# GuanxingLu/ManiGaussian

Measured on AMD Instinct MI355X. Metric: Gaussians rasterized/sec (fwd+bwd), 128x128, 32 feat-ch; HBM GB/s vs peak, higher is better.
Workload: dtype f32

## Files before the change

manigaussian_amd/csrc/mgs_render_dense.hip:

```cpp
#include "mgs_render_common.h"

namespace mgs {

constexpr int TRACE_EVENTS = 24;
__device__ unsigned long long g_trace[512 * 16 * TRACE_EVENTS];
#define MGS_TRACE(ev)                                                                                      \
  do {                                                                                                     \
    if ((r.dbg & 256) && lane == 0 && blockIdx.x < 512 && (ev) < TRACE_EVENTS)                              \
      g_trace[((size_t)blockIdx.x * 16 + w) * TRACE_EVENTS + (ev)] = __builtin_amdgcn_s_memtime();         \
  } while (0)

template <int F, bool FAST, bool EXACT, int NW, int CHS, bool TWO>
__global__ void __launch_bounds__(NW * 64, TWO ? 4 : 1)
coop_fwd_pairs_kernel(RenderArgs r, const uint2* __restrict__ ranges, const uint32_t* __restrict__ point_list,
                      float* __restrict__ T_end, float* __restrict__ T_mid,
                      uint32_t* __restrict__ last_pos, float* __restrict__ partial, uint32_t* __restrict__ surv,
                      size_t surv_stride, uint2* __restrict__ nsurv, float* __restrict__ final_T,
                      uint32_t* __restrict__ last_chunk, float* __restrict__ out_color, float* __restrict__ out_feat,
                      uint32_t* __restrict__ round_base, uint32_t pool, uint32_t* __restrict__ flags, int nblocks,
                      uint64_t* host_status, uint32_t status_tag, unsigned long long* hs_fail_mark) {
  static_assert(CHS == 64, "a chunk is two 32-lane groups of the Gaussian-major backward");
  using f32x16 = __attribute__((ext_vector_type(16))) float;
  constexpr int NCH = F + 3;
  constexpr bool MF = F >= 16;
  constexpr int NT = MF ? (F + 31) / 32 : 0;
  constexpr int NVF = MF ? 0 : F;
  constexpr int NP = NW / 2;
  constexpr int NS = 2;
  constexpr int NSTEP = CHS / 2;
  constexpr int TRS = 33;
  constexpr int NOWN = (NCH + NW - 1) / NW;
  constexpr uint32_t ROUND = NW * CHS;
  constexpr uint32_t FSTEP = NW * 64;
  constexpr int FILLK = 3;
  constexpr int TRR = NT * 32 + 3;
  __shared__ float trs[MF ? NW * TRR * TRS : 1];
  __shared__ uint32_t lastcc[NW];
  __shared__ float4 recP[NW][CHS / 4 * 2 * 3];
  __shared__ uint32_t sid[NW * CHS];
  __shared__ float4 rowq[NW][NS][CHS];
  __shared__ float rowf[NVF > 0 ? NW * NS * CHS * NVF : 1];
  __shared__ float Tp[2][NW][64];
  __shared__ unsigned long long red_last[64];
  __shared__ uint32_t cnt[2][FILLK * NW];
  __shared__ uint32_t rbase[2];
  constexpr uint32_t RBH = 16;
  __shared__ uint32_t rb_hist[RBH];
  const int tid = threadIdx.x, lane = tid & 63;
  const int w = __builtin_amdgcn_readfirstlane(tid >> 6);
  if (blockIdx.x == 0 && tid == 0 && hs_fail_mark) *hs_fail_mark = 0ull;
  const int pr = w >> 1, hh = w & 1;
  const int k_ = lane >> 5, pl_ = lane & 31;
  int tile, sub;
  map_block(blockIdx.x, tile, sub);
  if (tile >= r.tiles_x * r.tiles_y) return;
  const PixBlk p = pix_blk(r, tile, sub, lane);
  const int pixq_ = 32 * hh + pl_;
  const int pixq = pixq_, k = k_, pl = pl_;
  const PixBlk pq = pix_blk(r, tile, sub, pixq);
  const int pixx_ = 32 * (hh ^ k) + pl;
  const int pixx = pixx_;
  const bool insidex = pix_blk(r, tile, sub, pixx).inside;
  const uint2 rng = ranges[tile];
  const bool use_feat = (F > 0) && r.include_feature;
  const bool eager = (r.dbg & (1 << 17)) != 0;
  const auto feat_rsrc = __builtin_amdgcn_make_buffer_rsrc(const_cast<float*>(r.feats), 0, 0xffffffffu, 0x00020000);
  uint32_t* __restrict__ my_rounds = round_base + round_entry(rng.x, tile, sub, 0);
  bool overflow = false;
  uint32_t* my_surv = surv + (size_t)sub * surv_stride + rng.x;

  float Tround = 1.0f;
  uint32_t my_vis = 0;
  float my_Tf = 1.0f;
  if (w == 0) red_last[lane] = (unsigned long long)__float_as_uint(1.0f);
  uint32_t my_lastcc = 0xffffffffu;
  MGS_TRACE(0);

  uint32_t next = rng.x;
  uint32_t qhead = 0;
  uint32_t qtail = 0;
  uint32_t cbase = 0;
  uint32_t fill = 0;
  uint32_t round = 0;

  const bool allocator = tid == (NW - 1) * 64;
  const bool static0 = (uint32_t)nblocks <= 1024u && (uint32_t)nblocks * (uint32_t)NW <= pool;
  const uint32_t dyn_base = static0 ? (uint32_t)nblocks * (uint32_t)NW : 0u;
  for (;; round++) {
    int k = k_, pl = pl_, pixq = pixq_, pixx = pixx_;
    asm volatile("" : "+v"(k), "+v"(pl), "+v"(pixq), "+v"(pixx));
    uint32_t b0 = 0;
    const bool more = next < rng.y || qtail > qhead;
    if (allocator && more) {
      if (static0 && round == 0) b0 = ((uint32_t)tile * 4u + (uint32_t)sub) * (uint32_t)NW;
      else b0 = dyn_base + atomicAdd(&flags[FLAG_CHUNKS_USED], (uint32_t)NW);
    }
    while (qtail - qhead < ROUND && next < rng.y) {
      uint32_t idd[FILLK], rk[FILLK];
      float4 a0[FILLK], a1[FILLK];
      {
#pragma unroll
        for (int kf = 0; kf < FILLK; kf++) {
          const uint32_t e = next + (uint32_t)kf * FSTEP + (uint32_t)tid;
          idd[kf] = e < rng.y ? point_list[e] : 0xffffffffu;
        }
#pragma unroll
        for (int kf = 0; kf < FILLK; kf++) {
          a0[kf] = make_float4(0, 0, 0, 0); a1[kf] = make_float4(0, 0, -1.f, -1.f);
          if (idd[kf] != 0xffffffffu) { a0[kf] = r.rec[2 * (size_t)idd[kf]]; a1[kf] = r.rec[2 * (size_t)idd[kf] + 1]; }
        }
#pragma unroll
        for (int kf = 0; kf < FILLK; kf++) {
          const bool sk = idd[kf] != 0xffffffffu && cull_ok<EXACT>(a0[kf], a1[kf], p);
          const unsigned long long sm = ballot(sk);
          rk[kf] = sk ? (uint32_t)__builtin_popcountll(sm & ((1ull << lane) - 1ull)) : 0xffffffffu;
          if (lane == 0) cnt[fill & 1][kf * NW + w] = (uint32_t)__builtin_popcountll(sm);
        }
      }
      __syncthreads();
      const uint32_t v = lane < FILLK * NW ? cnt[fill & 1][lane] : 0u;
      const uint32_t incl = wave_incl_scan_add_u32(v);
      const uint32_t total = bcast_lane_u32(incl, 63);
#pragma unroll
      for (int kf = 0; kf < FILLK; kf++) {
        const uint32_t base = bcast_lane_u32(incl - v, kf * NW + w);
        if (rk[kf] != 0xffffffffu) {
          const uint32_t n = qtail + base + rk[kf];
          my_surv[n] = idd[kf];
          if (round == 0 && n < ROUND) {
            const uint32_t e = n & (CHS - 1);
            float* rp = reinterpret_cast<float*>(&recP[n / CHS][0]) + (((e >> 2) * 2 + (e & 1)) * 12 + ((e >> 1) & 1));
            rp[0] = a0[kf].x; rp[2] = a0[kf].y; rp[4] = a0[kf].z; rp[6] = a0[kf].w; rp[8] = a1[kf].x; rp[10] = a1[kf].y;
            sid[n] = idd[kf];
          }
        }
      }
      qtail += total;
      next += FILLK * FSTEP;
      fill++;
    }
    if (allocator && more) {
      rbase[round & 1] = b0;
      if (round < RBH) rb_hist[round] = b0;
      my_rounds[4 * (size_t)round] = b0;
    }
    MGS_TRACE(1 + 8 * round);
    __syncthreads();
    MGS_TRACE(2 + 8 * round);
    const uint32_t avail = qtail - qhead;
    const bool exhausted = !(next < rng.y);
    uint32_t nchunk = exhausted ? (avail + CHS - 1) / CHS : avail / CHS;
    nchunk = min(nchunk, (uint32_t)NW);
    if (nchunk == 0) break;

    struct Rec3 { float4 XY, CC, ZO; };
    auto rec3_of = [&](uint32_t buf, int j) -> Rec3 {
      return Rec3{recP[buf][(2 * j + k) * 3], recP[buf][(2 * j + k) * 3 + 1], recP[buf][(2 * j + k) * 3 + 2]};
    };
    auto alpha2_rec = [&](const Rec3& R) -> f32x2 {
      const float4 XY = R.XY, CC = R.CC, ZO = R.ZO;
      const f32x2 dx = f32x2{XY.x, XY.y} - pq.pxf, dy = f32x2{XY.z, XY.w} - pq.pyf;
      const f32x2 power = gauss_power2v(f32x2{CC.x, CC.y}, f32x2{CC.z, CC.w}, f32x2{ZO.x, ZO.y}, dx, dy);
      const f32x2 G = exp2_<FAST>(power);
      const f32x2 oG = f32x2{ZO.z, ZO.w} * G;
      const float a0 = fminf(0.99f, oG.x), a1 = fminf(0.99f, oG.y);
      return f32x2{((power.x > 0.0f) || (a0 < 1.0f / 255.0f)) ? 0.f : a0, ((power.y > 0.0f) || (a1 < 1.0f / 255.0f)) ? 0.f : a1};
    };
    float al[NSTEP];
    uint32_t nmy[NS];
#pragma unroll
    for (int q = 0; q < NS; q++) {
      const uint32_t ci = (uint32_t)pr + (uint32_t)q * NP;
      nmy[q] = ci < nchunk ? min((uint32_t)CHS, avail - ci * CHS) : 0u;
    }
    auto phase_a = [&](const int q, const bool publish) __attribute__((always_inline)) {
      const uint32_t ci = (uint32_t)pr + (uint32_t)q * NP;
      const bool hasq = ci < nchunk;
      float tp = 1.0f;
      if (hasq) {
        float4 rq = make_float4(0, 0, 0, __uint_as_float(0u));
        float fv[NVF > 0 ? NVF : 1];
#pragma unroll
        for (int i = 0; i < (NVF > 0 ? NVF : 1); i++) fv[i] = 0.f;
        const bool valid = (uint32_t)lane < (q ? nmy[1] : nmy[0]);
        float* rp = reinterpret_cast<float*>(&recP[ci][0]) + (((lane >> 2) * 2 + (lane & 1)) * 12 + ((lane >> 1) & 1));
        int tile_ = tile;
        asm volatile("" : "+s"(tile_));
        const uint32_t gbase = gauss_base(r, tile_);
        auto colour_row = [&](uint32_t id) {
          const uint32_t gid = gauss_of(gbase, id);
          const uint32_t cid = r.colors_per_view ? id : gid;
          rq = make_float4(r.colors[(size_t)cid * 3], r.colors[(size_t)cid * 3 + 1], r.colors[(size_t)cid * 3 + 2],
                           __uint_as_float(gid));
          if constexpr (NVF > 0) {
            if (use_feat) {
#pragma unroll
              for (int i = 0; i < NVF; i++) fv[i] = r.feats[(size_t)gid * F + i];
            }
          }
        };
        if (round == 0) {
          if (valid) {
            colour_row(sid[ci * CHS + (uint32_t)lane]);
          } else {
            rp[0] = 0.f; rp[2] = 0.f; rp[4] = 0.f; rp[6] = 0.f; rp[8] = 0.f; rp[10] = 0.f;
            rq.w = __uint_as_float(gauss_of(gbase, sid[ci * CHS]));
          }
        } else {
          float4 g0 = make_float4(0, 0, 0, 0), g1 = make_float4(0, 0, -1.f, -1.f);
          if (valid) {
            const uint32_t id = my_surv[qhead + ci * CHS + (uint32_t)lane];
            g0 = r.rec[2 * (size_t)id]; g1 = r.rec[2 * (size_t)id + 1];
            colour_row(id);
          } else {
            rq.w = __uint_as_float(gauss_of(gbase, my_surv[qhead + ci * CHS]));
          }
          rp[0] = g0.x; rp[2] = g0.y; rp[4] = g0.z; rp[6] = g0.w; rp[8] = g1.x;
          rp[10] = valid ? g1.y : 0.f;
        }
        wave_lds_sync();
        if (q == 0) MGS_TRACE(3 + 8 * round);
        f32x2 tp2 = {1.0f, 1.0f};
        Rec3 Rn = rec3_of(ci, 0);
#pragma unroll
        for (int j = 0; j < NSTEP / 2; j++) {
          const Rec3 Rc = Rn;
          if (j + 1 < NSTEP / 2) Rn = rec3_of(ci, j + 1);
          const f32x2 a2 = alpha2_rec(Rc);
          al[2 * j] = a2.x; al[2 * j + 1] = a2.y;
          tp2 = tp2 * (1.0f - a2);
        }
        tp = tp2.x * tp2.y;
        rowq[w][q][lane] = rq;
        if constexpr (NVF > 0) {
#pragma unroll
          for (int i = 0; i < NVF; i++) rowf[(((size_t)w * NS + q) * CHS + lane) * NVF + i] = fv[i];
        }
        float t0 = tp, t1 = tp;
        swap32(t0, t1);
        tp = t0 * t1;
      }
      if (publish && k == 0) Tp[round & 1][ci][pixq] = tp;
    };
    uint32_t rb = 0;
    auto phase_b = [&](const int q, const float Tin_q) __attribute__((always_inline)) {
      const uint32_t ci = (uint32_t)pr + (uint32_t)q * NP;
      const bool hasq = ci < nchunk;
      const float Tpart = __uint_as_float(lane_xor<32>(__float_as_uint(Tin_q), lane));
      float T = k ? Tpart : Tin_q;
      const bool live = hasq && pq.inside && !(T < 0.0001f);
      if (ballot(live) != 0) {
        const uint32_t n_my = q ? nmy[1] : nmy[0];
        float Cc[3] = {0.f, 0.f, 0.f};
        float Cv[NVF > 0 ? NVF : 1];
#pragma unroll
        for (int i = 0; i < (NVF > 0 ? NVF : 1); i++) Cv[i] = 0.f;
        f32x16 acc[NT > 0 ? NT : 1];
#pragma unroll
        for (int t = 0; t < (NT > 0 ? NT : 1); t++)
#pragma unroll
          for (int i = 0; i < 16; i++) acc[t][i] = 0.f;
        constexpr int BD = 4;
        float Bq[NT > 0 ? NT : 1][BD];
        uint32_t gnext = __float_as_uint(rowq[w][q][k].w);
        auto load_B = [&](int s) {
          const uint32_t gide = gnext;
          if (s + 1 < NSTEP) gnext = __float_as_uint(rowq[w][q][2 * (s + 1) + k].w);
#pragma unroll
          for (int t = 0; t < (NT > 0 ? NT : 1); t++) {
            const int ch = 32 * t + pl;
            if constexpr (MF)
              Bq[t][s % BD] = __uint_as_float(__builtin_amdgcn_raw_buffer_load_b32(
                  feat_rsrc, gide * (uint32_t)(F * 4) + (uint32_t)((ch < F ? ch : 0) * 4), 0, 0));
          }
        };
        if constexpr (MF) {
#pragma unroll
          for (int s = 0; s < BD; s++) load_B(s);
        }
        float Tc = live ? T : 0.f;
        uint32_t last = 0;
        float Tm = T;
        bool stop = false;
        constexpr int GS = 4;
#pragma unroll
        for (int g = 0; g < NSTEP / GS; g++) {
          if (g * GS == NSTEP / 2) Tm = T;
          stop = stop || (uint32_t)(2 * g * GS) >= n_my || ballot(Tc != 0.f) == 0;
          __builtin_amdgcn_sched_barrier(0);
          if (!stop) {
#pragma unroll
            for (int u4 = 0; u4 < GS; u4++) {
              const int s = g * GS + u4;
              float a0 = al[s], a1 = a0;
              swap32(a0, a1);
              float wq[2];
              const float aa[2] = {a0, a1};
#pragma unroll
              for (int u = 0; u < 2; u++) {
                const float test_T = Tc * (1.0f - aa[u]);
                const bool term = test_T < 0.0001f;
                wq[u] = (term ? 0.f : aa[u]) * Tc;
                Tc = term ? 0.f : test_T;
                T = term ? T : test_T;
                last = wq[u] > 0.f ? (uint32_t)(2 * s + u) + 1u : last;
              }
              const float wk = k ? wq[1] : wq[0];
              const float4 rq = rowq[w][q][2 * s + k];
              Cc[0] += rq.x * wk; Cc[1] += rq.y * wk; Cc[2] += rq.z * wk;
              if constexpr (NVF > 0) {
#pragma unroll
                for (int i = 0; i < NVF; i++) Cv[i] += rowf[(((size_t)w * NS + q) * CHS + 2 * s + k) * NVF + i] * wk;
              }
              if constexpr (MF) {
#pragma unroll
                for (int t = 0; t < NT; t++) {
                  float bv = Bq[t][s % BD];
                  if constexpr (F % 32 != 0) bv = (32 * t + pl) < F ? bv : 0.f;
                  acc[t] = __builtin_amdgcn_mfma_f32_32x32x2f32(wk, bv, acc[t], 0, 0, 0);
                }
                if (s + BD < NSTEP) load_B(s + BD);
              }
            }
          }
        }
        if constexpr (MF) {
#pragma unroll
          for (int t = 0; t < NT; t++)
#pragma unroll
            for (int i = 0; i < BD; i++) asm volatile("" ::"v"(Bq[t][i]));
        }
        if (last <= 32u) Tm = T;
#pragma unroll
        for (int i = 0; i < 3; i++) Cc[i] += __uint_as_float(lane_xor<32>(__float_as_uint(Cc[i]), lane));
#pragma unroll
        for (int i = 0; i < NVF; i++) Cv[i] += __uint_as_float(lane_xor<32>(__float_as_uint(Cv[i]), lane));
        MGS_TRACE(6 + 8 * round);
        const size_t slot = (size_t)rb + (size_t)ci;
        float* pp = partial + slot * NCH * 64 + pixq;
        if (k == 0) {
          T_end[slot * 64 + pixq] = T;
          T_mid[slot * 64 + pixq] = Tm;
          last_pos[slot * 64 + pixq] = last;
#pragma unroll
          for (int i = 0; i < 3; i++) pp[i * 64] = Cc[i];
#pragma unroll
          for (int i = 0; i < NVF; i++) pp[(3 + i) * 64] = Cv[i];
        }
        if constexpr (MF) {
          float* tb = trs + (size_t)w * TRR * TRS;
#pragma unroll
          for (int t = 0; t < NT; t++)
#pragma unroll
            for (int i = 0; i < 16; i++)
              tb[(32 * t + pl) * TRS + (i & 3) + 8 * (i >> 2) + 4 * k] = acc[t][i];
          if (k == 0) {
#pragma unroll
            for (int i = 0; i < 3; i++) tb[(NT * 32 + i) * TRS + pl] = Cc[i];
          }
          wave_lds_sync();
#pragma unroll
          for (int c = 0; c < F / 2; c++) {
            const int ch = k * (F / 2) + c;
            pp[(3 + ch) * 64] = tb[ch * TRS + pl];
          }
          wave_lds_sync();
          my_lastcc = cbase + ci;
        }
        if (live) { my_vis = cbase + ci + 1; my_Tf = T; }
      }
    };
    constexpr int GA = 2;
    static_assert(GA < NP, "slot 1 goes in two groups of pairs");
    float Tnext = Tround;
    int p0 = 0, p1 = NP;
#pragma clang loop unroll(disable)
    for (int st = eager ? -1 : 0;; st++) {
      asm volatile("" : "+v"(k), "+v"(pl), "+v"(pixq), "+v"(pixx));
      const int q = st == 0 ? 0 : 1;
      const bool act = pr >= p0 && pr < p1;
#pragma unroll
      for (int s = 0; s < NSTEP; s++) al[s] = 0.f;
      if (act) {
        phase_a(q, st <= 0 || !eager);
        if (st > 0) MGS_TRACE(8 + 8 * round);
      }
      if (st < 0) continue;
      if (st == 0) MGS_TRACE(4 + 8 * round);
      if (st == 0 || !eager) __syncthreads();
      if (st == 0) {
        __builtin_amdgcn_s_waitcnt(0x0F70);
        MGS_TRACE(5 + 8 * round);
        rb = rbase[round & 1];
        if (rb + (uint32_t)NW > pool) { overflow = true; break; }
      }
      float Tin = Tnext;
#pragma unroll
      for (int c2 = 0; c2 < NP; c2++) {
        const float t2 = (c2 >= p0 && c2 < p1) ? Tp[round & 1][q * NP + c2][pixx] : 1.0f;
        Tin = (c2 < pr) ? Tin * t2 : Tin;
        Tnext *= t2;
      }
      if (act) phase_b(q, Tin);
      if (st == 2) break;
      p0 = st == 0 ? 0 : GA;
      p1 = st == 0 ? GA : NP;
      if (!((uint32_t)(NP + p0) < nchunk) || ballot(insidex && !(Tnext < 0.0001f)) == 0) break;
    }
    if (overflow) break;
    MGS_TRACE(7 + 8 * round);
    Tround = Tnext;
    qhead += min(avail, nchunk * CHS);
    cbase += nchunk;
    if (ballot(insidex && !(Tround < 0.0001f)) == 0) break;
  }

  MGS_TRACE(TRACE_EVENTS - 3);
  if (my_vis > 0 && k == 0)
    atomicMax(&red_last[pixq], ((unsigned long long)my_vis << 32) | (unsigned long long)__float_as_uint(my_Tf));
  if constexpr (MF) { if (lane == 0) lastcc[w] = my_lastcc; }
  __syncthreads();
  const unsigned long long rl = red_last[lane];
  const uint32_t vis = (uint32_t)(rl >> 32);
  const float Tf = __uint_as_float((uint32_t)rl);
  float img[NOWN];
#pragma unroll
  for (int kk = 0; kk < NOWN; kk++) img[kk] = 0.f;
  const uint32_t vmax = wave_umax(vis);
  constexpr int NFLY = 8;
  static_assert(NW % NFLY == 0, "a batch of the final sum lies inside one round");
  for (uint32_t c0 = 0; c0 < vmax; c0 += NFLY) {
    float v[NFLY][NOWN];
    const uint32_t rr = c0 / NW;
    uint32_t rb0 = rb_hist[rr < RBH ? rr : 0u];
    if (__builtin_expect(rr >= RBH, 0))
      rb0 = __hip_atomic_load(&my_rounds[4 * (size_t)rr], __ATOMIC_RELAXED, __HIP_MEMORY_SCOPE_WORKGROUP);
    rb0 = (uint32_t)__builtin_amdgcn_readfirstlane((int)rb0);
    bool inl[NFLY];
    unsigned long long needg = 0ull;
#pragma unroll
    for (int u = 0; u < NFLY; u++) {
      const uint32_t cc = c0 + u;
      inl[u] = false;
      if constexpr (MF) {
        const uint32_t ws = 2u * ((cc % NW) % NP) + (uint32_t)(lane >> 5);
        inl[u] = lastcc[ws] == cc;
      }
      needg |= ballot(cc < vis && !inl[u]);
#pragma unroll
      for (int kk = 0; kk < NOWN; kk++) v[u][kk] = 0.f;
    }
    if (needg != 0ull) {
#pragma unroll
      for (int u = 0; u < NFLY; u++) {
        const uint32_t cc = c0 + u;
        const bool gl = cc < vis && !inl[u];
        const size_t slot = gl ? (size_t)rb0 + (cc % NW) : 0;
        const float* pp = partial + slot * NCH * 64 + lane;
#pragma unroll
        for (int kk = 0; kk < NOWN; kk++) {
          const int ch = w + kk * NW;
          if (gl && ch < NCH && (ch < 3 || use_feat)) v[u][kk] = pp[ch * 64];
        }
      }
#pragma unroll
      for (int u = 0; u < NFLY; u++)
#pragma unroll
        for (int kk = 0; kk < NOWN; kk++) asm volatile("" : "+v"(v[u][kk]));
    }
    if constexpr (MF) {
#pragma unroll
      for (int u = 0; u < NFLY; u++) {
        const uint32_t cc = c0 + u;
        const uint32_t ws = 2u * ((cc % NW) % NP) + (uint32_t)(lane >> 5);
        const float* tb = trs + (size_t)ws * TRR * TRS + (lane & 31);
#pragma unroll
        for (int kk = 0; kk < NOWN; kk++) {
          const int ch = w + kk * NW;
          const int row = ch < 3 ? NT * 32 + ch : ch - 3;
          if (cc < vis && inl[u] && ch < NCH && (ch < 3 || use_feat)) v[u][kk] = tb[row * TRS];
        }
      }
    }
#pragma unroll
    for (int u = 0; u < NFLY; u++)
#pragma unroll
      for (int kk = 0; kk < NOWN; kk++) img[kk] += v[u][kk];
  }
  MGS_TRACE(TRACE_EVENTS - 2);
  uint32_t ticket = 0;
  if (tid == 0) {
    const uint32_t dep = overflow ? (atomicOr(&flags[FLAG_PREFILTERED], 0x100u) & 0u) : 0u;
    ticket = atomicAdd(&flags[FLAG_BLOCKS_DONE], 1u + dep) + 1u;
  }
  const size_t HW = (size_t)r.Hv * r.W;
  int lane_o = lane;
  asm volatile("" : "+v"(lane_o));
  const PixBlk po = pix_blk(r, tile, sub, lane_o);
  if (po.inside) {
#pragma unroll
    for (int kk = 0; kk < NOWN; kk++) {
      const int ch = w + kk * NW;
      if (ch < 3) out_color[((size_t)po.v * 3 + ch) * HW + po.pixl] = img[kk] + Tf * r.bg[ch];
      else if (ch < NCH && use_feat) out_feat[((size_t)po.v * F + (ch - 3)) * HW + po.pixl] = img[kk];
    }
  }
  if (w == 0) {
    last_chunk[((size_t)tile * 4 + sub) * 64 + lane] = vis;
    if (po.inside) final_T[po.pixa] = Tf;
    if (lane == 0) {
      nsurv[(size_t)tile * 4 + sub] = make_uint2(qtail, round > 0 || vis > 0 ? rb_hist[0] : 0u);
      if (ticket == (uint32_t)nblocks && host_status) {
        const uint32_t used = dyn_base + __hip_atomic_load(&flags[FLAG_CHUNKS_USED], __ATOMIC_RELAXED, __HIP_MEMORY_SCOPE_AGENT);
        const uint32_t ovf = (__hip_atomic_load(&flags[FLAG_PREFILTERED], __ATOMIC_RELAXED, __HIP_MEMORY_SCOPE_AGENT) >> 8) & 1u;
        __hip_atomic_store(host_status + 1, ((uint64_t)(status_tag & 0xffffu) << 48) | ((uint64_t)ovf << 32) | used,
                           __ATOMIC_RELEASE, __HIP_MEMORY_SCOPE_SYSTEM);
      }
    }
  }
  MGS_TRACE(TRACE_EVENTS - 1);
}

template <int F>
static hipError_t dense_F(const RenderArgs& r, const BinView& b, const ImgView& im, const ChunkView& cv, float* oc,
                          float* of, StatusSink st, hipStream_t s) {
  const int T = r.tiles_x * r.tiles_y;
  const int grid = ((T + 7) / 8) * 32;
#define MGS_CFD_(FAST, EXACT, NW, TWO)                                                                                \
  hipLaunchKernelGGL((coop_fwd_pairs_kernel<F, FAST, EXACT, NW, CHUNK, TWO>), dim3(grid), dim3(NW * 64), 0, s, r,      \
                     im.ranges, b.point_list, cv.T_end, cv.T_mid, cv.last_pos, cv.partial, cv.surv,                   \
                     cv.surv_stride, cv.nsurv, im.final_T, cv.last_chunk, oc, of, cv.round_base, cv.pool, im.flags,   \
                     4 * T, st.host, st.tag, (im.direct_keys && im.ready) ? im.ready + 1 : nullptr)
#define MGS_CFD(FAST, EXACT)                                                                                          \
  do {                                                                                                                \
    if constexpr (F > 32) MGS_CFD_(FAST, EXACT, 8, false);                               \
    else if (r.nwf == 8) MGS_CFD_(FAST, EXACT, 8, true);                                    \
    else MGS_CFD_(FAST, EXACT, 16, false);                                                                            \
  } while (0)
  if (r.fast_exp) { if (r.exact_cull) MGS_CFD(true, true); else MGS_CFD(true, false); }
  else            { if (r.exact_cull) MGS_CFD(false, true); else MGS_CFD(false, false); }
#undef MGS_CFD
#undef MGS_CFD_
  return hipGetLastError();
}

hipError_t launch_render_fwd_dense(const RenderArgs& r, const BinView& b, const ImgView& im, const ChunkView& cv,
                                   float* out_color, float* out_feat, StatusSink st, hipStream_t s) {
  const int F = r.include_feature ? r.F : 0;
  switch (F) {
#define X(N) case N: return dense_F<N>(r, b, im, cv, out_color, out_feat, st, s);
    MGS_FOR_EACH_F(X)
#undef X
    default: return hipErrorInvalidValue;
  }
}

}

extern "C" int mgs_debug_read_trace(unsigned long long* host, size_t count) {
  const size_t n = sizeof(mgs::g_trace) / sizeof(unsigned long long);
  return (int)hipMemcpyFromSymbol(host, HIP_SYMBOL(mgs::g_trace), (count < n ? count : n) * sizeof(unsigned long long));
}
```

Measured before the change: 765.5 million.

## Keep second-slot chunk partials in LDS and issue LDS reads unconditionally in final sum

```diff
diff --git a/manigaussian_amd/csrc/mgs_render_dense.hip b/manigaussian_amd/csrc/mgs_render_dense.hip
--- a/manigaussian_amd/csrc/mgs_render_dense.hip
+++ b/manigaussian_amd/csrc/mgs_render_dense.hip
@@ -34,8 +34,11 @@
   constexpr uint32_t FSTEP = NW * 64;
   constexpr int FILLK = 3;
   constexpr int TRR = NT * 32 + 3;
-  __shared__ float trs[MF ? NW * TRR * TRS : 1];
-  __shared__ uint32_t lastcc[NW];
+  constexpr int GA = 2;
+  constexpr bool KEEP = MF && !TWO;
+  constexpr int NHB = KEEP ? NW + 2 * GA : NW;
+  __shared__ float trs[MF ? NHB * TRR * TRS : 1];
+  __shared__ uint32_t lastcc[KEEP ? 2 * NW : NW];
   __shared__ float4 recP[NW][CHS / 4 * 2 * 3];
   __shared__ uint32_t sid[NW * CHS];
   __shared__ float4 rowq[NW][NS][CHS];
@@ -73,7 +76,8 @@
   uint32_t my_vis = 0;
   float my_Tf = 1.0f;
   if (w == 0) red_last[lane] = (unsigned long long)__float_as_uint(1.0f);
-  uint32_t my_lastcc = 0xffffffffu;
+  uint32_t my_lastcc = 0xffffffffu, my_lastcc2 = 0xffffffffu;
+  const bool keep = KEEP && (r.dbg & (1 << 18)) == 0;
   MGS_TRACE(0);
 
   uint32_t next = rng.x;
@@ -348,7 +352,8 @@
           for (int i = 0; i < NVF; i++) pp[(3 + i) * 64] = Cv[i];
         }
         if constexpr (MF) {
-          float* tb = trs + (size_t)w * TRR * TRS;
+          const bool second = keep && q == 1 && pr < GA;
+          float* tb = trs + (size_t)(second ? NW + w : w) * TRR * TRS;
 #pragma unroll
           for (int t = 0; t < NT; t++)
 #pragma unroll
@@ -365,12 +370,11 @@
             pp[(3 + ch) * 64] = tb[ch * TRS + pl];
           }
           wave_lds_sync();
-          my_lastcc = cbase + ci;
+          if (second) my_lastcc2 = cbase + ci; else my_lastcc = cbase + ci;
         }
         if (live) { my_vis = cbase + ci + 1; my_Tf = T; }
       }
     };
-    constexpr int GA = 2;
     static_assert(GA < NP, "slot 1 goes in two groups of pairs");
     float Tnext = Tround;
     int p0 = 0, p1 = NP;
@@ -418,7 +422,12 @@
   MGS_TRACE(TRACE_EVENTS - 3);
   if (my_vis > 0 && k == 0)
     atomicMax(&red_last[pixq], ((unsigned long long)my_vis << 32) | (unsigned long long)__float_as_uint(my_Tf));
-  if constexpr (MF) { if (lane == 0) lastcc[w] = my_lastcc; }
+  if constexpr (MF) {
+    if (lane == 0) {
+      lastcc[w] = my_lastcc;
+      if constexpr (KEEP) lastcc[NW + w] = my_lastcc2;
+    }
+  }
   __syncthreads();
   const unsigned long long rl = red_last[lane];
   const uint32_t vis = (uint32_t)(rl >> 32);
@@ -427,8 +436,14 @@
 #pragma unroll
   for (int kk = 0; kk < NOWN; kk++) img[kk] = 0.f;
   const uint32_t vmax = wave_umax(vis);
-  constexpr int NFLY = 8;
+  constexpr int NFLY = NOWN > 4 ? 4 : 8;
   static_assert(NW % NFLY == 0, "a batch of the final sum lies inside one round");
+  static_assert(NFLY % NP == 0, "chunk c0 + u of a batch was blended by pair u % NP (NP divides NW, NFLY divides c0)");
+  auto own = [&](int kk) { const int ch = w + kk * NW; return ch < NCH && (ch < 3 || use_feat); };
+  auto hrow = [&](int kk) {
+    const int ch = w + kk * NW;
+    return (uint32_t)(lane >> 5) * (TRR * TRS) + (uint32_t)((ch < 3 ? NT * 32 + ch : ch < NCH ? ch - 3 : 0) * TRS) + (uint32_t)(lane & 31);
+  };
   for (uint32_t c0 = 0; c0 < vmax; c0 += NFLY) {
     float v[NFLY][NOWN];
     const uint32_t rr = c0 / NW;
@@ -436,15 +451,18 @@
     if (__builtin_expect(rr >= RBH, 0))
       rb0 = __hip_atomic_load(&my_rounds[4 * (size_t)rr], __ATOMIC_RELAXED, __HIP_MEMORY_SCOPE_WORKGROUP);
     rb0 = (uint32_t)__builtin_amdgcn_readfirstlane((int)rb0);
-    bool inl[NFLY];
+    bool inl[NFLY], in2[NFLY];
     unsigned long long needg = 0ull;
 #pragma unroll
     for (int u = 0; u < NFLY; u++) {
       const uint32_t cc = c0 + u;
-      inl[u] = false;
+      inl[u] = in2[u] = false;
       if constexpr (MF) {
-        const uint32_t ws = 2u * ((cc % NW) % NP) + (uint32_t)(lane >> 5);
-        inl[u] = lastcc[ws] == cc;
+        const uint32_t ws = 2u * (uint32_t)(u % NP) + (uint32_t)(lane >> 5);
+        if constexpr (KEEP) {
+          if ((u % NP) < GA) in2[u] = lastcc[NW + ws] == cc;
+        }
+        inl[u] = in2[u] || lastcc[ws] == cc;
       }
       needg |= ballot(cc < vis && !inl[u]);
 #pragma unroll
@@ -469,17 +487,23 @@
         for (int kk = 0; kk < NOWN; kk++) asm volatile("" : "+v"(v[u][kk]));
     }
     if constexpr (MF) {
+      float x[NFLY][NOWN];
+#pragma unroll
+      for (int u = 0; u < NFLY; u++)
+#pragma unroll
+        for (int kk = 0; kk < NOWN; kk++) {
+          const uint32_t at = hrow(kk) + (uint32_t)(2 * (u % NP) * TRR * TRS);
+          x[u][kk] = trs[(KEEP && (u % NP) < GA && in2[u]) ? at + (uint32_t)(NW * TRR * TRS) : at];
+        }
+#pragma unroll
+      for (int u = 0; u < NFLY; u++)
+#pragma unroll
+        for (int kk = 0; kk < NOWN; kk++) asm volatile("" : "+v"(x[u][kk]));
 #pragma unroll
       for (int u = 0; u < NFLY; u++) {
-        const uint32_t cc = c0 + u;
-        const uint32_t ws = 2u * ((cc % NW) % NP) + (uint32_t)(lane >> 5);
-        const float* tb = trs + (size_t)ws * TRR * TRS + (lane & 31);
-#pragma unroll
-        for (int kk = 0; kk < NOWN; kk++) {
-          const int ch = w + kk * NW;
-          const int row = ch < 3 ? NT * 32 + ch : ch - 3;
-          if (cc < vis && inl[u] && ch < NCH && (ch < 3 || use_feat)) v[u][kk] = tb[row * TRS];
-        }
+        const bool take = c0 + u < vis && inl[u];
+#pragma unroll
+        for (int kk = 0; kk < NOWN; kk++) v[u][kk] = (take && own(kk)) ? x[u][kk] : v[u][kk];
       }
     }
 #pragma unroll
```

Measured after the change: 769.8 million (median of 2 runs). No clear change (+0.6%).

## Park first-round slot-1 tiles in extra LDS and restructure the final reduction

Applied to the files above, without the earlier changes.

```diff
diff --git a/manigaussian_amd/csrc/mgs_render_dense.hip b/manigaussian_amd/csrc/mgs_render_dense.hip
--- a/manigaussian_amd/csrc/mgs_render_dense.hip
+++ b/manigaussian_amd/csrc/mgs_render_dense.hip
@@ -46,6 +46,12 @@
   __shared__ uint32_t rbase[2];
   constexpr uint32_t RBH = 16;
   __shared__ uint32_t rb_hist[RBH];
+  constexpr int GA = 2;
+  constexpr bool PARK = MF && !TWO;
+  constexpr int NPK = 2 * GA;
+  __shared__ float trs2[PARK ? NPK * TRR * TRS : 1];
+  __shared__ uint32_t parkcc[NPK];
+  constexpr int OLD_TAIL = 1 << 18;
   const int tid = threadIdx.x, lane = tid & 63;
   const int w = __builtin_amdgcn_readfirstlane(tid >> 6);
   if (blockIdx.x == 0 && tid == 0 && hs_fail_mark) *hs_fail_mark = 0ull;
@@ -73,6 +79,8 @@
   uint32_t my_vis = 0;
   float my_Tf = 1.0f;
   if (w == 0) red_last[lane] = (unsigned long long)__float_as_uint(1.0f);
+  if (PARK && tid < NPK) parkcc[tid] = 0xffffffffu;
+  const float bgw = w < 3 ? r.bg[w] : 0.f;
   uint32_t my_lastcc = 0xffffffffu;
   MGS_TRACE(0);
 
@@ -348,7 +356,8 @@
           for (int i = 0; i < NVF; i++) pp[(3 + i) * 64] = Cv[i];
         }
         if constexpr (MF) {
-          float* tb = trs + (size_t)w * TRR * TRS;
+          const bool park = PARK && q == 1 && round == 0 && pr < GA && !(r.dbg & OLD_TAIL);
+          float* tb = park ? trs2 + (size_t)w * TRR * TRS : trs + (size_t)w * TRR * TRS;
 #pragma unroll
           for (int t = 0; t < NT; t++)
 #pragma unroll
@@ -365,12 +374,12 @@
             pp[(3 + ch) * 64] = tb[ch * TRS + pl];
           }
           wave_lds_sync();
-          my_lastcc = cbase + ci;
+          if (!park) my_lastcc = cbase + ci;
+          else if (lane == 0) parkcc[w] = cbase + ci;
         }
         if (live) { my_vis = cbase + ci + 1; my_Tf = T; }
       }
     };
-    constexpr int GA = 2;
     static_assert(GA < NP, "slot 1 goes in two groups of pairs");
     float Tnext = Tround;
     int p0 = 0, p1 = NP;
@@ -426,35 +435,31 @@
   float img[NOWN];
 #pragma unroll
   for (int kk = 0; kk < NOWN; kk++) img[kk] = 0.f;
-  const uint32_t vmax = wave_umax(vis);
+  const uint32_t vmax = (uint32_t)__builtin_amdgcn_readfirstlane((int)wave_umax(vis));
   constexpr int NFLY = 8;
   static_assert(NW % NFLY == 0, "a batch of the final sum lies inside one round");
-  for (uint32_t c0 = 0; c0 < vmax; c0 += NFLY) {
+  auto sum_batch = [&](const uint32_t c0, const uint32_t rb0) __attribute__((always_inline)) {
     float v[NFLY][NOWN];
-    const uint32_t rr = c0 / NW;
-    uint32_t rb0 = rb_hist[rr < RBH ? rr : 0u];
-    if (__builtin_expect(rr >= RBH, 0))
-      rb0 = __hip_atomic_load(&my_rounds[4 * (size_t)rr], __ATOMIC_RELAXED, __HIP_MEMORY_SCOPE_WORKGROUP);
-    rb0 = (uint32_t)__builtin_amdgcn_readfirstlane((int)rb0);
-    bool inl[NFLY];
-    unsigned long long needg = 0ull;
-#pragma unroll
-    for (int u = 0; u < NFLY; u++) {
-      const uint32_t cc = c0 + u;
-      inl[u] = false;
-      if constexpr (MF) {
-        const uint32_t ws = 2u * ((cc % NW) % NP) + (uint32_t)(lane >> 5);
-        inl[u] = lastcc[ws] == cc;
-      }
-      needg |= ballot(cc < vis && !inl[u]);
+    uint32_t m1 = 0, m2 = 0;
+    if constexpr (MF) {
+      const uint32_t cu = c0 + (uint32_t)(lane & 7);
+      const uint32_t wl = 2u * ((cu % NW) % NP) + (uint32_t)((lane >> 3) & 1);
+      const uint32_t sh = (uint32_t)(lane >> 5) * 8u;
+      m1 = ((uint32_t)ballot(lane < 16 && lastcc[wl] == cu) >> sh) & 0xffu;
+      if constexpr (PARK)
+        m2 = ((uint32_t)ballot(lane < 16 && (cu % NW) % NP < (uint32_t)GA && parkcc[wl < (uint32_t)NPK ? wl : 0u] == cu) >> sh) & 0xffu;
+    }
+    const uint32_t vm = (1u << (vis > c0 ? min(vis - c0, (uint32_t)NFLY) : 0u)) - 1u;
+    const uint32_t have = vm & (m1 | m2), need = vm & ~(m1 | m2);
+#pragma unroll
+    for (int u = 0; u < NFLY; u++)
 #pragma unroll
       for (int kk = 0; kk < NOWN; kk++) v[u][kk] = 0.f;
-    }
-    if (needg != 0ull) {
+    if (ballot(need != 0u) != 0ull) {
 #pragma unroll
       for (int u = 0; u < NFLY; u++) {
         const uint32_t cc = c0 + u;
-        const bool gl = cc < vis && !inl[u];
+        const bool gl = (need >> u) & 1u;
         const size_t slot = gl ? (size_t)rb0 + (cc % NW) : 0;
         const float* pp = partial + slot * NCH * 64 + lane;
 #pragma unroll
@@ -472,13 +477,19 @@
 #pragma unroll
       for (int u = 0; u < NFLY; u++) {
         const uint32_t cc = c0 + u;
-        const uint32_t ws = 2u * ((cc % NW) % NP) + (uint32_t)(lane >> 5);
-        const float* tb = trs + (size_t)ws * TRR * TRS + (lane & 31);
-#pragma unroll
-        for (int kk = 0; kk < NOWN; kk++) {
-          const int ch = w + kk * NW;
-          const int row = ch < 3 ? NT * 32 + ch : ch - 3;
-          if (cc < vis && inl[u] && ch < NCH && (ch < 3 || use_feat)) v[u][kk] = tb[row * TRS];
+        if (cc < vmax) {
+          const uint32_t ws = 2u * ((cc % NW) % NP) + (uint32_t)(lane >> 5);
+          const float* tb = (((m2 >> u) & 1u) ? trs2 : trs) + (size_t)ws * TRR * TRS + (lane & 31);
+          const bool hv = (have >> u) & 1u;
+#pragma unroll
+          for (int kk = 0; kk < NOWN; kk++) {
+            const int ch = w + kk * NW;
+            const int row = ch < 3 ? NT * 32 + ch : ch - 3;
+            if (ch < NCH) {
+              const float t = tb[row * TRS];
+              v[u][kk] = hv ? t : v[u][kk];
+            }
+          }
         }
       }
     }
@@ -486,12 +497,22 @@
     for (int u = 0; u < NFLY; u++)
 #pragma unroll
       for (int kk = 0; kk < NOWN; kk++) img[kk] += v[u][kk];
-  }
+  };
+  const uint32_t vhot = min(vmax, RBH * (uint32_t)NW);
+  for (uint32_t c0 = 0; c0 < vhot; c0 += NFLY)
+    sum_batch(c0, (uint32_t)__builtin_amdgcn_readfirstlane((int)rb_hist[c0 / NW]));
+  for (uint32_t c0 = RBH * (uint32_t)NW; c0 < vmax; c0 += NFLY)
+    sum_batch(c0, (uint32_t)__builtin_amdgcn_readfirstlane((int)__hip_atomic_load(
+                      &my_rounds[4 * (size_t)(c0 / NW)], __ATOMIC_RELAXED, __HIP_MEMORY_SCOPE_WORKGROUP)));
   MGS_TRACE(TRACE_EVENTS - 2);
+  const int tw = (r.dbg & OLD_TAIL) ? 0 : NW - 1;
   uint32_t ticket = 0;
-  if (tid == 0) {
+  if (tid == tw * 64) {
     const uint32_t dep = overflow ? (atomicOr(&flags[FLAG_PREFILTERED], 0x100u) & 0u) : 0u;
-    ticket = atomicAdd(&flags[FLAG_BLOCKS_DONE], 1u + dep) + 1u;
+    uint32_t done = FLAG_BLOCKS_DONE;
+    asm volatile("" : "+v"(done));
+    ticket = atomicAdd(&flags[done], 1u + dep);
+    if (r.dbg & OLD_TAIL) __builtin_amdgcn_s_waitcnt(0x0F70);
   }
   const size_t HW = (size_t)r.Hv * r.W;
   int lane_o = lane;
@@ -501,7 +522,7 @@
 #pragma unroll
     for (int kk = 0; kk < NOWN; kk++) {
       const int ch = w + kk * NW;
-      if (ch < 3) out_color[((size_t)po.v * 3 + ch) * HW + po.pixl] = img[kk] + Tf * r.bg[ch];
+      if (ch < 3) out_color[((size_t)po.v * 3 + ch) * HW + po.pixl] = img[kk] + Tf * bgw;
       else if (ch < NCH && use_feat) out_feat[((size_t)po.v * F + (ch - 3)) * HW + po.pixl] = img[kk];
     }
   }
@@ -510,12 +531,15 @@
     if (po.inside) final_T[po.pixa] = Tf;
     if (lane == 0) {
       nsurv[(size_t)tile * 4 + sub] = make_uint2(qtail, round > 0 || vis > 0 ? rb_hist[0] : 0u);
-      if (ticket == (uint32_t)nblocks && host_status) {
-        const uint32_t used = dyn_base + __hip_atomic_load(&flags[FLAG_CHUNKS_USED], __ATOMIC_RELAXED, __HIP_MEMORY_SCOPE_AGENT);
-        const uint32_t ovf = (__hip_atomic_load(&flags[FLAG_PREFILTERED], __ATOMIC_RELAXED, __HIP_MEMORY_SCOPE_AGENT) >> 8) & 1u;
-        __hip_atomic_store(host_status + 1, ((uint64_t)(status_tag & 0xffffu) << 48) | ((uint64_t)ovf << 32) | used,
-                           __ATOMIC_RELEASE, __HIP_MEMORY_SCOPE_SYSTEM);
-      }
+    }
+  }
+  if (tid == tw * 64) {
+    asm volatile("" : "+v"(ticket));
+    if (ticket + 1u == (uint32_t)nblocks && host_status) {
+      const uint32_t used = dyn_base + __hip_atomic_load(&flags[FLAG_CHUNKS_USED], __ATOMIC_RELAXED, __HIP_MEMORY_SCOPE_AGENT);
+      const uint32_t ovf = (__hip_atomic_load(&flags[FLAG_PREFILTERED], __ATOMIC_RELAXED, __HIP_MEMORY_SCOPE_AGENT) >> 8) & 1u;
+      __hip_atomic_store(host_status + 1, ((uint64_t)(status_tag & 0xffffu) << 48) | ((uint64_t)ovf << 32) | used,
+                         __ATOMIC_RELEASE, __HIP_MEMORY_SCOPE_SYSTEM);
     }
   }
   MGS_TRACE(TRACE_EVENTS - 1);
```

Result: no change. 765.0 million before, 766.7 million after, median of 3 (+0.2%).
